# gonglixue/RAFT-tf

Hardware: AMD Instinct MI355X
Metric: frames/sec (whole node), raft-things 2x436x1024, 32 iters, inference (higher is better)
Workload: dtype bf16; 1 GPU; model=raft-things, global_batch=1, height=436, width=1024, iters=32, parallelism=dp1, device=mi355x

## Files before the change

raft_amd/models/fused.py:

```python
from __future__ import annotations

from typing import Optional

import torch

ACT_NONE, ACT_RELU, ACT_SIGMOID, ACT_TANH = 0, 1, 2, 3


def _pad8(c: int) -> int:
    return (c + 7) // 8 * 8


def pack_conv(conv: torch.nn.Conv2d, pad_cin: Optional[int] = None,
              scale: float = 1.0):
    w = conv.weight.detach().float()
    N, Cin, kh, kw = w.shape
    cp = pad_cin if pad_cin is not None else Cin
    wp = w.new_zeros(N, cp, kh, kw)
    wp[:, :Cin] = w * scale
    wp = wp.permute(2, 3, 0, 1).reshape(kh * kw, N, cp)
    wp = wp.contiguous().to(device=conv.weight.device, dtype=torch.bfloat16)
    if conv.bias is not None:
        bias = (conv.bias.detach().float() * scale).contiguous()
    else:
# ... 9 lines not shown


class _FC:

    def __init__(self, conv, pad_cin=None, scale=1.0):
        self.wp, self.bias, self.kh, self.kw = pack_conv(conv, pad_cin, scale)

    def __call__(self, hip, in1, in2=None, act=ACT_RELU, out=None, n_off=0,
                 in1_off=0, in1_len=0, stride=1, res=None):
        return hip.fconv_plain(in1, in2, self.wp, self.bias, self.kh,
                               self.kw, act, out, n_off, in1_off, in1_len,
                               -1, -1, stride, res)


class _GruDir:
    def __init__(self, convz, convr, convq):
        self.zr_w, self.zr_b, self.kh, self.kw = pack_zr(convz, convr)
        self.q_w, self.q_b, _, _ = pack_conv(convq)

    def __call__(self, hip, h, x):
        z, rh = hip.fconv_gru_zr(h, x, self.zr_w, self.zr_b, self.kh, self.kw)
        return hip.fconv_gru_q(rh, x, self.q_w, self.q_b, self.kh, self.kw,
                               z, h)


def _pack_fp8(wp_bf16, dev):
    w = wp_bf16.float()
    aw = float(w.abs().max().clamp_min(1e-12))
    w8 = (w * (448.0 / aw)).to(torch.float8_e4m3fn).view(torch.uint8)
    return w8.contiguous().to(dev), aw


class _GruDirFP8:

    def __init__(self, convz, convr, convq):
        zr_w, self.zr_b, self.kh, self.kw = pack_zr(convz, convr)
        q_w, self.q_b, _, _ = pack_conv(convq)
        dev = self.zr_b.device
        self.zr_w8, self.zr_aw = _pack_fp8(zr_w, dev)
        self.q_w8, self.q_aw = _pack_fp8(q_w, dev)

    def __call__(self, hip, h, x8, ax, h8):
        z, rh8 = hip.fconv_fp8_gru_zr(h8, x8, h, self.zr_w8, self.zr_b, ax,
                                      self.zr_aw, self.kh, self.kw)
        return hip.fconv_fp8_gru_q(rh8, x8, self.q_w8, self.q_b, ax,
                                   self.q_aw, self.kh, self.kw, z, h)


class FusedBasicUpdate:

    def __init__(self, ub, corr_cpad: int, ctx_dim: int):
        enc = ub.encoder
        self.c1 = _FC(enc.convc1, pad_cin=corr_cpad)
        self.c2 = _FC(enc.convc2)
        self.f1 = _FC(enc.convf1)
        self.f2 = _FC(enc.convf2)
        self.cv = _FC(enc.conv)
        import os as _os
        hd = ub.gru.convz1.weight.shape[0]
        cat_dim = ub.gru.convz1.weight.shape[1]
        self.fp8_gru = (_os.environ.get("RAFT_AMD_FP8_GRU", "0") == "1"
                        and hd % 128 == 0 and (cat_dim - hd) % 128 == 0)
        if self.fp8_gru:
            self.gru1 = _GruDirFP8(ub.gru.convz1, ub.gru.convr1,
                                   ub.gru.convq1)
            self.gru2 = _GruDirFP8(ub.gru.convz2, ub.gru.convr2,
                                   ub.gru.convq2)
        else:
            self.gru1 = _GruDir(ub.gru.convz1, ub.gru.convr1, ub.gru.convq1)
            self.gru2 = _GruDir(ub.gru.convz2, ub.gru.convr2, ub.gru.convq2)
        self.fh1 = _FC(ub.flow_head.conv1)
        self.m0 = _FC(ub.mask[0])
        self.heads_w = torch.cat([self.fh1.wp, self.m0.wp], dim=1) \
            .contiguous()
        self.heads_b = torch.cat([self.fh1.bias, self.m0.bias]).contiguous()
        self.fh2 = _FC(ub.flow_head.conv2)
        self.m2 = _FC(ub.mask[2], scale=0.25)
        self.ctx_dim = ctx_dim
        self.side_stream = None
        self._ev_fork = torch.cuda.Event()
        self._ev_join = torch.cuda.Event()

    def __call__(self, hip, net, x_buf, corr_pad, coords1, final=True):
        ctx = self.ctx_dim
        side = self.side_stream
        if side is not None and not torch.cuda.is_current_stream_capturing():
            cur = torch.cuda.current_stream()
            self._ev_fork.record(cur)
            side.wait_event(self._ev_fork)
            with torch.cuda.stream(side):
                flo1 = hip.fconv_smallk(x_buf, self.f1.wp, self.f1.bias,
                                        self.f1.kh, self.f1.kw, ACT_RELU,
                                        ctx + 126, 2, 1)
                flo = self.f2(hip, flo1)
                self._ev_join.record(side)
            cor = self.c2(hip, self.c1(hip, corr_pad))
            cur.wait_event(self._ev_join)
            flo.record_stream(cur)
        else:
            cor = self.c2(hip, self.c1(hip, corr_pad))
            flo1 = hip.fconv_smallk(x_buf, self.f1.wp, self.f1.bias,
                                    self.f1.kh, self.f1.kw, ACT_RELU,
                                    ctx + 126, 2, 1)
            flo = self.f2(hip, flo1)
        self.cv(hip, cor, flo, ACT_RELU, out=x_buf, n_off=ctx)
        if self.fp8_gru:
            ax = x_buf.abs().amax().to(torch.float32).clamp_(min=1.0) \
                .contiguous()
            x8 = hip.quant_fp8(x_buf, ax)
            net = self.gru1(hip, net, x8, ax, hip.quant_fp8(net, ax))
            net = self.gru2(hip, net, x8, ax, hip.quant_fp8(net, ax))
        else:
            net = self.gru1(hip, net, x_buf)
            net = self.gru2(hip, net, x_buf)
        if not final:
            h1 = self.fh1(hip, net)
            coords_new = hip.fconv_dflow_coords(h1, self.fh2.wp,
                                                self.fh2.bias, coords1, 3, 3)
            return net, None, coords_new
        hbuf = hip.fconv_plain(net, None, self.heads_w, self.heads_b, 3, 3,
                               ACT_RELU, None, 0, 0, 0, -1, -1, 1, None)
        coords_new = hip.fconv_dflow_coords(hbuf, self.fh2.wp,
                                            self.fh2.bias, coords1, 3, 3)
        mask = self.m2(hip, hbuf, act=ACT_NONE, in1_off=256, in1_len=256)
        return net, mask, coords_new


class FusedSmallUpdate:

    def __init__(self, ub, corr_cpad: int, ctx_dim: int):
        enc = ub.encoder
        self.c1 = _FC(enc.convc1, pad_cin=corr_cpad)
        self.f1 = _FC(enc.convf1)
        self.f2 = _FC(enc.convf2)
        self.cv = _FC(enc.conv)
        self.gru = _GruDir(ub.gru.convz, ub.gru.convr, ub.gru.convq)
        self.fh1 = _FC(ub.flow_head.conv1)
        self.fh2 = _FC(ub.flow_head.conv2)
        self.ctx_dim = ctx_dim
        self.side_stream = None
        self._ev_fork = torch.cuda.Event()
        self._ev_join = torch.cuda.Event()

    def __call__(self, hip, net, x_buf, corr_pad, coords1, final=True):
        ctx = self.ctx_dim
        side = self.side_stream
        if side is not None and not torch.cuda.is_current_stream_capturing():
            cur = torch.cuda.current_stream()
            self._ev_fork.record(cur)
            side.wait_event(self._ev_fork)
            with torch.cuda.stream(side):
                flo1 = hip.fconv_smallk(x_buf, self.f1.wp, self.f1.bias,
                                        self.f1.kh, self.f1.kw, ACT_RELU,
                                        ctx + 80, 2, 1)
                flo = self.f2(hip, flo1)
                self._ev_join.record(side)
            cor = self.c1(hip, corr_pad)
            cur.wait_event(self._ev_join)
            flo.record_stream(cur)
        else:
            cor = self.c1(hip, corr_pad)
            flo1 = hip.fconv_smallk(x_buf, self.f1.wp, self.f1.bias,
                                    self.f1.kh, self.f1.kw, ACT_RELU,
                                    ctx + 80, 2, 1)
            flo = self.f2(hip, flo1)
        self.cv(hip, cor, flo, ACT_RELU, out=x_buf, n_off=ctx)
        net = self.gru(hip, net, x_buf)
        h1 = self.fh1(hip, net)
        coords_new = hip.fconv_dflow_coords(h1, self.fh2.wp, self.fh2.bias,
                                            coords1, 3, 3)
        return net, None, coords_new


def pack_raw(w: torch.Tensor, bias, pad_cin: Optional[int] = None):
    N, Cin, kh, kw = w.shape
    cp = pad_cin if pad_cin is not None else Cin
    wp = w.new_zeros(N, cp, kh, kw)
    wp[:, :Cin] = w
    wp = wp.permute(2, 3, 0, 1).reshape(kh * kw, N, cp)
    wp = wp.contiguous().to(torch.bfloat16)
    if bias is None:
        bias = torch.zeros(N, device=w.device)
# ... 98 lines not shown


_warned_bidir_fp8 = False


class FusedRaft:

    def __init__(self, model):
        from raft_amd.ops import require_hip
        self.hip = require_hip()
        self.model = model
        cfg = model.cfg
        K = 2 * cfg.corr_radius + 1
        self.corr_c = cfg.corr_levels * K * K
        self.corr_cpad = _pad8(self.corr_c)
        if cfg.small:
            self.update = FusedSmallUpdate(model.update_block, self.corr_cpad,
                                           cfg.context_dim)
            self.x_dim = cfg.context_dim + 82
        else:
            self.update = FusedBasicUpdate(model.update_block, self.corr_cpad,
                                           cfg.context_dim)
            self.x_dim = cfg.context_dim + 128
        import os
        self.fuse_enc = os.environ.get("RAFT_AMD_EAGER_ENC", "0") != "1"
        if self.fuse_enc:
            fnorm = "instance"
            cnorm = "none" if cfg.small else "batch"
            self.fnet_f = FusedEncoder(model.fnet, fnorm)
            self.cnet_f = FusedEncoder(model.cnet, cnorm)
        self._version = self._weights_version()
        self._graphs = {}

    def _weights_version(self) -> int:
        return sum(p._version for p in self.model.parameters())

    def stale(self) -> bool:
        return self._version != self._weights_version()

    @torch.no_grad()
    def _loop(self, levels, net, x_buf, coords0, coords1, iters):
        cfg = self.model.cfg
        hip = self.hip
        B, H8, W8, _ = coords0.shape
        corr_buf = torch.zeros(B, H8, W8, self.corr_cpad,
                               device=net.device, dtype=torch.bfloat16)
        flow_off = self.x_dim - 2
        mask = None
        for it in range(iters):
            corr_pad = hip.corr_lookup_nhwc(list(levels), coords1,
                                            cfg.corr_radius, self.corr_cpad,
                                            True, corr_buf, x_buf, flow_off,
                                            getattr(self, "_vol_scale",
                                                    None))
            net, mask, coords1 = self.update(hip, net, x_buf, corr_pad,
                                             coords1,
                                             final=(it == iters - 1))

        flow = coords1 - coords0
        if cfg.small:
            from raft_amd.ops import torch_ref
            up = torch_ref.upflow8(flow.permute(0, 3, 1, 2))
            if cfg.scale_small_upflow:
                up = 8.0 * up
            return up, flow
        flow_nchw = flow.permute(0, 3, 1, 2).contiguous()
        mask_nchw = mask.permute(0, 3, 1, 2).contiguous()
        return hip.convex_upsample(flow_nchw, mask_nchw), flow

    def _side(self):
        side = getattr(self, "_side_stream", None)
        if side is None:
# ... 221 lines not shown
```

raft_amd/ops/csrc/bindings.cpp:

```cpp
#include <torch/extension.h>

#include <ATen/hip/HIPContext.h>
#include <c10/hip/HIPStream.h>
#include <hip/hip_runtime_api.h>

#include <cmath>
#include <vector>

extern "C" {
void launch_corr_volume_f32(const float*, const float*, float*, int, int,
                            int, int, float, hipStream_t);
void launch_corr_pool2x_f32(const float*, float*, int, int, int, int,
                            long long, hipStream_t);
void launch_corr_lookup_fwd_f32(const float* const*, const int*, const int*,
                                const float*, float*, int, int, int, int,
                                int, hipStream_t);
void launch_corr_lookup_bwd_f32(float* const*, const int*, const int*,
                                const float*, const float*, int, int, int,
                                int, int, hipStream_t);
void launch_corr_lookup_bwd_wave_f32(float* const*, const int*, const int*,
                                     const float*, const void*, int, int,
                                     int, int, int, int, int, hipStream_t);
void launch_gru_gates_fwd_f32(const float*, const float*, const float*,
                              float*, long long, hipStream_t);
// ... 43 lines not shown
int launch_frame_interp(const float*, const float*, const float*,
                        const float*, const unsigned char*,
                        const unsigned char*, unsigned long long*, float*,
                        float*, float*, unsigned char*, int, int, int, int,
                        float, hipStream_t);
void launch_corr_lookup_nhwc(const void* const*, const int*, const int*,
                             int, const float*, const float*, void*, bool,
                             void*, int, int, int, int, int, int, int, int,
                             hipStream_t);
void launch_corr_lookup_nhwc_bwd(float* const*, const int*, const int*,
                                 const float*, const float*, int, int, int,
                                 int, int, hipStream_t);
void launch_corr_pool2x_bf16(const void*, void*, int, int, int, int,
                             long long, hipStream_t);
void launch_fconv_nhwc_bf16(const void*, int, int, int, const void*, int,
                            const void*, const float*, void*, int, int, int,
                            int, int, int, int, int, int, int, const void*,
                            const void*, void*, void*, int, int, int,
                            hipStream_t);
void launch_inorm_stats(const void*, float*, float*, float*, int, int,
                        int, float, hipStream_t);
int inorm_stats_partitions(int);
void launch_inorm_apply(const void*, const float*, const float*,
                        const void*, void*, int, int, int, int,
                        hipStream_t);
void launch_fconv_smallk_nhwc_bf16(const void*, int, int, const void*,
                                   const float*, void*, int, int, int, int,
                                   int, int, int, int, int, hipStream_t);
void launch_fconv_dflow_coords(const void*, int, int, int, const void*,
                               const float*, const float*, float*, int, int,
                               int, int, int, hipStream_t);
}

// ... 626 lines not shown
        res_ptr = res->data_ptr();
        mode = 3;
    }
    at::Tensor out;
    int cstride;
    if (out_buf.has_value()) {
        out = out_buf.value();
        CHECK_CONT(out);
        cstride = out.size(3);
    } else {
        out = at::empty({B, Ho, Wo, N}, in1.options());
        cstride = N;
        n_off = 0;
    }
    launch_fconv_nhwc_bf16(in1.data_ptr(), C1, in1_stride, (int)in1_off,
                           p2, C2, wp.data_ptr(), bptr, out.data_ptr(), B,
                           Ho, Wo, N, (int)n_off, cstride, (int)kh, (int)kw,
                           (int)act, mode, res_ptr, nullptr, nullptr,
                           nullptr, (int)alltaps, (int)mtiles, (int)stride,
                           current_stream());
    return out;
}

std::vector<at::Tensor> fconv_gru_zr(at::Tensor h, at::Tensor x,
                                     at::Tensor wp, at::Tensor bias,
                                     int64_t kh, int64_t kw) {
    CHECK_DEV(h); CHECK_CONT(h); CHECK_CONT(x); CHECK_CONT(wp);
    const int B = h.size(0), H = h.size(1), W = h.size(2), hd = h.size(3);
    const int N = wp.size(1);
    TORCH_CHECK(N == 2 * hd, "zr weights must stack [Wz; Wr]");
    auto z = at::empty_like(h);
    auto rh = at::empty_like(h);
    launch_fconv_nhwc_bf16(h.data_ptr(), hd, hd, 0, x.data_ptr(),
                           x.size(3), wp.data_ptr(), bias.data_ptr<float>(),
                           nullptr, B, H, W, N, 0, 0, (int)kh, (int)kw, 0,
                           1, h.data_ptr(), nullptr, z.data_ptr(),
                           rh.data_ptr(), -1, -1, 1, current_stream());
    return {z, rh};
}

at::Tensor fconv_gru_q(at::Tensor rh, at::Tensor x, at::Tensor wp,
                       at::Tensor bias, int64_t kh, int64_t kw, at::Tensor z,
                       at::Tensor h) {
    CHECK_DEV(rh); CHECK_CONT(rh); CHECK_CONT(x); CHECK_CONT(wp);
    CHECK_CONT(z); CHECK_CONT(h);
    const int B = rh.size(0), H = rh.size(1), W = rh.size(2);
    const int hd = rh.size(3);
    TORCH_CHECK(wp.size(1) == hd);
    auto out = at::empty_like(h);
    launch_fconv_nhwc_bf16(rh.data_ptr(), hd, hd, 0, x.data_ptr(),
                           x.size(3), wp.data_ptr(),
                           bias.data_ptr<float>(), out.data_ptr(), B, H, W,
                           hd, 0, hd, (int)kh, (int)kw, 0, 2, h.data_ptr(),
                           z.data_ptr(), nullptr, nullptr, -1, -1, 1,
                           current_stream());
    return out;
}

at::Tensor fconv_smallk(at::Tensor in1, at::Tensor wp,
                        c10::optional<at::Tensor> bias, int64_t kh,
                        int64_t kw, int64_t act, int64_t in1_off,
                        int64_t in1_len, int64_t conv_stride) {
    CHECK_DEV(in1); CHECK_CONT(in1); CHECK_CONT(wp);
    const int B = in1.size(0), H = in1.size(1), W = in1.size(2);
    const int stride = in1.size(3);
    const int C = in1_len > 0 ? (int)in1_len : stride;
    const int N = wp.size(1);
    const float* bptr = bias.has_value() ? bias->data_ptr<float>() : nullptr;
    const int Ho = (int)(H / conv_stride), Wo = (int)(W / conv_stride);
    TORCH_CHECK(conv_stride == 1 ||
// ... 98 lines not shown
          py::arg("levels"), py::arg("coords"), py::arg("radius"),
          py::arg("c_stride"), py::arg("out_bf16"),
          py::arg("out_buf") = c10::nullopt,
          py::arg("flow_buf") = c10::nullopt, py::arg("flow_off") = 0,
          py::arg("vol_scale") = c10::nullopt);
    m.def("fconv_plain", &fconv_plain,
          "fused NHWC bf16 conv (+bias +activation, slice output)");
    m.def("fconv_gru_zr", &fconv_gru_zr, "GRU z/r gate conv pair");
    m.def("fconv_smallk", &fconv_smallk, "direct NHWC conv for tiny Cin");
    m.def("inorm_stats", &inorm_stats, "per-(b,c) instance-norm stats");
    m.def("inorm_apply", &inorm_apply,
          "instance-norm apply (+relu / +residual-relu)");
    m.def("fconv_dflow_coords", &fconv_dflow_coords,
          "flow-head final conv fused with the coords update");
    m.def("fconv_gru_q", &fconv_gru_q, "GRU candidate conv + state update");
}
```

raft_amd/ops/csrc/fconv.hip:

```cpp

#include "common.h"
#include "fconv_dispatch.h"
#include <hip/hip_bf16.h>
#include <cstdio>

typedef short short8 __attribute__((ext_vector_type(8)));
typedef unsigned int uint4v __attribute__((ext_vector_type(4)));

#define FC_BM 64
#define FC_BN 128
#define FC_BK 32
#define FC_ROWB (FC_BK * 2)

RAFT_DEV unsigned fswz(int row, unsigned colbyte) {
    return (unsigned)(row * FC_ROWB + colbyte) ^
           (((unsigned)row & 3u) << 4) ^ ((((unsigned)row >> 2) & 3u) << 6);
}

RAFT_DEV float factivate(float v, int act) {
    if (act == 1) return fmaxf(v, 0.0f);
    if (act == 2) return 1.0f / (1.0f + __expf(-v));
    if (act == 3) return tanhf(v);
    return v;
}

#define EP_PLAIN 0
#define EP_GRU_ZR 1
#define EP_GRU_Q 2
#define EP_RES_RELU 3

template <int KH, int KW, int MI, int NJ, bool AT, int MT, int S, int TH = 1,
          bool PIPE = false>
__global__ __launch_bounds__(256) void fconv_nhwc_bf16_k(
    const __hip_bfloat16* __restrict__ in1, int C1,
    int in1_stride, int in1_off,
    const __hip_bfloat16* __restrict__ in2, int C2,
    const __hip_bfloat16* __restrict__ wp,
    const float* __restrict__ bias,
    __hip_bfloat16* __restrict__ out,
    int H, int W, int N, int n_off, int out_cstride, int act, int mode,
    const __hip_bfloat16* __restrict__ h_state,
    const __hip_bfloat16* __restrict__ z_buf_in,
    __hip_bfloat16* __restrict__ z_buf_out,
    __hip_bfloat16* __restrict__ rh_out) {
    constexpr int TAPS = KH * KW;
    constexpr int BM = 32 * MI;
    constexpr int BN = 32 * NJ;
    constexpr int PAR = (S == 2) ? 2 : 1;
    constexpr int PBW = (S == 2) ? (KW - 2) / 2 : KW / 2;
    constexpr int PBH = (S == 2) ? (KH - 2) / 2 : KH / 2;
    constexpr int RLO = (S == 2) ? (PBW + 1) / 2 : 0;
    constexpr int BMX = BM / TH;
    constexpr int AW = (S == 2) ? (BM + RLO + (KW + 1) / 2 + 1)
                                : (BMX + KW - 1);
    constexpr int APAD = ((AW + 15) / 16) * 16;
    constexpr int NSLAB = ((AT ? KH : 1) + TH - 1) * MT * PAR;
    constexpr int NBT = AT ? TAPS : KW;
    constexpr int ABYTES = APAD * FC_ROWB;
    constexpr int BBYTES = BN * FC_ROWB;
// ... 10 lines not shown
    const int wave = tid >> 6;
    const int wm = (wave >> 1) * (16 * MI);
    const int wn = (wave & 1) * (16 * NJ);
    const long long HW = (long long)H * W;
    const int ksteps = (Cin + FC_BK - 1) / FC_BK;
    const int nsteps = AT ? ksteps : KH * ksteps;

    floatx4 acc[MT][MI][NJ];
#pragma unroll
    for (int mt = 0; mt < MT; ++mt)
#pragma unroll
        for (int i = 0; i < MI; ++i)
#pragma unroll
            for (int j = 0; j < NJ; ++j)
                acc[mt][i][j] = {0.f, 0.f, 0.f, 0.f};

    char* const sAbase = smem;
    char* const sBbase = smem + NSLAB * ABYTES;

    auto stage = [&](int s) {
        const int ty0 = AT ? 0 : s / ksteps;
        const int k0 = (AT ? s : (s - ty0 * ksteps)) * FC_BK;
        const int Hi = (S == 2) ? 2 * H : H;
        const int Wi = (S == 2) ? 2 * W : W;
        const bool a_one = (k0 + FC_BK <= C1) || (k0 >= C1);
        const bool a_rows =
            (S == 1) && (y - KH / 2 + (AT ? 0 : ty0) >= 0) &&
            (y + (AT ? KH - 1 : ty0) + TH - 1 - KH / 2 < H);
        const bool a_cols = (x0 - KW / 2 + (MT - 1) * 0 >= 0) &&
                            (x0 + MT * BMX - 1 + (KW - 1) / 2 < W);
        if (a_one && a_rows && a_cols && S == 1) {
            const bool use1 = k0 + FC_BK <= C1;
            const __hip_bfloat16* src = use1 ? in1 : in2;
            const int cs = use1 ? in1_stride : C2;
            const int co = use1 ? (in1_off + k0) : (k0 - C1);
            for (int e = tid; e < NSLAB * AW * (FC_BK / 8); e += 256) {
                const int sl = e / (AW * (FC_BK / 8));
                const int rem0 = e % (AW * (FC_BK / 8));
                const int ar = rem0 / (FC_BK / 8);
                const int c8 = (rem0 % (FC_BK / 8)) * 8;
                const int mt = (sl / PAR) % MT;
                const int rsl = sl / (PAR * MT);
                const int row = y + (ty0 + rsl) - PBH;
                const int x = x0 + mt * BMX + ar - PBW;
                const uint4v v = *(const uint4v*)(
                    src + (((long long)b * H + row) * W + x) * cs + co + c8);
                *(uint4v*)(sAbase + sl * ABYTES + fswz(ar, c8 * 2)) = v;
            }
        } else
// ... 14 lines not shown
                : (x0 + mt * BMX + ar - PBW);
            uint4v v = {0, 0, 0, 0};
            if (row_ok && x >= 0 && x < Wi) {
                const int k = k0 + c8;
                const long long p = ((long long)b * Hi + row) * Wi + x;
                if (k < C1) {
                    if (k + 8 <= C1)
                        v = *(const uint4v*)(in1 + p * in1_stride + in1_off
                                             + k);
                    else {
                        __hip_bfloat16 tmp[8];
                        for (int u = 0; u < 8; ++u) {
                            const int kk = k + u;
                            tmp[u] = (kk < C1)
                                   ? in1[p * in1_stride + in1_off + kk]
                                   : (kk - C1 < C2 ? in2[p * C2 + kk - C1]
                                                   : (__hip_bfloat16)0.f);
                        }
                        v = *(const uint4v*)tmp;
                    }
                } else if (k - C1 < C2) {
                    if (k - C1 + 8 <= C2)
                        v = *(const uint4v*)(in2 + p * C2 + (k - C1));
                    else {
                        __hip_bfloat16 tmp[8];
                        for (int u = 0; u < 8; ++u) {
                            const int kk = k - C1 + u;
                            tmp[u] = kk < C2 ? in2[p * C2 + kk]
                                             : (__hip_bfloat16)0.f;
                        }
                        v = *(const uint4v*)tmp;
                    }
                }
            }
            *(uint4v*)(sA + fswz(ar, c8 * 2)) = v;
        }
        if (n0 + BN <= N && k0 + FC_BK <= Cin) {
            for (int e = tid; e < NBT * BN * (FC_BK / 8); e += 256) {
                const int t = e / (BN * (FC_BK / 8));
                const int rem = e % (BN * (FC_BK / 8));
                const int n = rem / (FC_BK / 8);
                const int c8 = (rem % (FC_BK / 8)) * 8;
                const int tap = AT ? t : (ty0 * KW + t);
// ... 81 lines not shown

        auto loadA = [&](int s, uint4v* rg) {
            const int ty0 = AT ? 0 : s / ksteps;
            const int k0 = (AT ? s : (s - ty0 * ksteps)) * FC_BK;
            const int Hi = (S == 2) ? 2 * H : H;
            const int Wi = (S == 2) ? 2 * W : W;
            const bool a_one = (k0 + FC_BK <= C1) || (k0 >= C1);
            const bool a_rows =
                (S == 1) && (y - KH / 2 + (AT ? 0 : ty0) >= 0) &&
                (y + (AT ? KH - 1 : ty0) + TH - 1 - KH / 2 < H);
            const bool a_cols = (x0 - KW / 2 >= 0) &&
                                (x0 + MT * BMX - 1 + (KW - 1) / 2 < W);
            if (S == 1 && a_one && a_rows && a_cols) {
                const bool use1 = k0 + FC_BK <= C1;
                const __hip_bfloat16* src = use1 ? in1 : in2;
                const int cs = use1 ? in1_stride : C2;
                const int co = use1 ? (in1_off + k0) : (k0 - C1);
#pragma unroll
                for (int r = 0; r < RA; ++r) {
                    const int e = tid + r * 256;
                    if (e < TOTA) {
                        const int sl = e / (AW * (FC_BK / 8));
                        const int rem0 = e % (AW * (FC_BK / 8));
                        const int ar = rem0 / (FC_BK / 8);
                        const int c8 = (rem0 % (FC_BK / 8)) * 8;
                        const int mt = (sl / PAR) % MT;
                        const int rsl = sl / (PAR * MT);
                        const int row = y + (ty0 + rsl) - PBH;
                        const int x = x0 + mt * BMX + ar - PBW;
                        rg[r] = *(const uint4v*)(
                            src + (((long long)b * H + row) * W + x) * cs +
// ... 22 lines not shown
                        : (x0 + mt * BMX + ar - PBW);
                    if (row_ok && x >= 0 && x < Wi) {
                        const int k = k0 + c8;
                        const long long p = ((long long)b * Hi + row) * Wi + x;
                        if (k < C1) {
                            if (k + 8 <= C1)
                                v = *(const uint4v*)(
                                    in1 + p * in1_stride + in1_off + k);
                            else {
                                __hip_bfloat16 tmp[8];
                                for (int u = 0; u < 8; ++u) {
                                    const int kk = k + u;
                                    tmp[u] = (kk < C1)
                                        ? in1[p * in1_stride + in1_off + kk]
                                        : (kk - C1 < C2
                                               ? in2[p * C2 + kk - C1]
                                               : (__hip_bfloat16)0.f);
                                }
                                v = *(const uint4v*)tmp;
                            }
                        } else if (k - C1 < C2) {
                            if (k - C1 + 8 <= C2)
                                v = *(const uint4v*)(in2 + p * C2 + (k - C1));
                            else {
                                __hip_bfloat16 tmp[8];
                                for (int u = 0; u < 8; ++u) {
                                    const int kk = k - C1 + u;
                                    tmp[u] = kk < C2
                                        ? in2[p * C2 + kk]
                                        : (__hip_bfloat16)0.f;
                                }
                                v = *(const uint4v*)tmp;
                            }
                        }
                    }
                }
                rg[r] = v;
            }
        };

        auto loadB = [&](int s, uint4v* rg) {
            const int ty0 = AT ? 0 : s / ksteps;
            const int k0 = (AT ? s : (s - ty0 * ksteps)) * FC_BK;
            if (n0 + BN <= N && k0 + FC_BK <= Cin) {
// ... 92 lines not shown
                const int m = wm + i * 16 + (lane >> 4) * 4 + r;
                const int n = n0 + wn + j * 16 + (lane & 15);
                const int yy2 = y + m / BMX;
                const int x = x0 + mt * BMX + m % BMX;
                if (x >= W || n >= N || yy2 >= H) continue;
                const long long p = ((long long)b * H + yy2) * W + x;
                float v = acc[mt][i][j][r];
                if (bias) v += bias[n];
                if (mode == EP_PLAIN) {
                    out[p * out_cstride + n_off + n] =
                        (__hip_bfloat16)factivate(v, act);
                } else if (mode == EP_RES_RELU) {
                    const float res = (float)h_state[p * hd + n];
                    out[p * out_cstride + n_off + n] = (__hip_bfloat16)
                        fmaxf(res + fmaxf(v, 0.0f), 0.0f);
                } else if (mode == EP_GRU_ZR) {
                    const float s = 1.0f / (1.0f + __expf(-v));
                    if (n < hd) {
                        z_buf_out[p * hd + n] = (__hip_bfloat16)s;
                    } else {
                        const int c = n - hd;
                        rh_out[p * hd + c] = (__hip_bfloat16)(
                            s * (float)h_state[p * hd + c]);
                    }
                } else {
                    const float q = tanhf(v);
                    const float z = (float)z_buf_in[p * hd + n];
                    const float h = (float)h_state[p * hd + n];
                    out[p * out_cstride + n_off + n] =
                        (__hip_bfloat16)((1.0f - z) * h + z * q);
                }
            }
}


extern "C" __global__ __launch_bounds__(256) void fconv_stem_s2_k(
    const __hip_bfloat16* __restrict__ in,
    const __hip_bfloat16* __restrict__ wp,
    const float* __restrict__ bias,
    __hip_bfloat16* __restrict__ out,
    int H, int W, int N, int act) {
    constexpr int KT = 49, KTP = 52;
// ... 186 lines not shown
}

static const FconvKnobs& fconv_knobs() {
    static const FconvKnobs k = fconv_knobs_from_env();
    return k;
}

struct FconvArgs {
    const __hip_bfloat16 *in1, *in2, *wp;
    const float* bias;
    __hip_bfloat16* out;
    const __hip_bfloat16 *h_state, *z_buf_in;
    __hip_bfloat16 *z_buf_out, *rh_out;
    int act;
    hipStream_t s;
};

template <int KH, int KW, int MI, int NJ, bool AT, int MT, int S, int TH,
          bool PIPE>
static bool fc_try(const FconvPick& p, const FconvShape& sh,
                   const FconvArgs& a) {
    if (p.KH != KH || p.KW != KW || p.MI != MI || p.NJ != NJ ||
        (p.AT != 0) != AT || p.MT != MT || p.S != S || p.TH != TH ||
        (p.PIPE != 0) != PIPE)
        return false;
    unsigned g[3];
    fconv_generic_grid(p, sh, g);
    hipLaunchKernelGGL(
        (fconv_nhwc_bf16_k<KH, KW, MI, NJ, AT, MT, S, TH, PIPE>),
        dim3(g[0], g[1], g[2]), dim3(256), 0, a.s, a.in1, sh.C1,
        sh.in1_stride, sh.in1_off, a.in2, sh.C2, a.wp, a.bias, a.out, sh.H,
        sh.W, sh.N, sh.n_off, sh.out_cstride, a.act, sh.mode, a.h_state,
        a.z_buf_in, a.z_buf_out, a.rh_out);
    return true;
}

template <int KH, int KW, int MI, int NJ, bool AT, int MT, int S, int TH>
static bool fc_try_pp(const FconvPick& p, const FconvShape& sh,
                      const FconvArgs& a) {
    return fc_try<KH, KW, MI, NJ, AT, MT, S, TH, false>(p, sh, a) ||
           fc_try<KH, KW, MI, NJ, AT, MT, S, TH, true>(p, sh, a);
}

template <int KH, int KW>
static bool fc_try_s1(const FconvPick& p, const FconvShape& sh,
                      const FconvArgs& a) {
    if (p.S != 1 || p.KH != KH || p.KW != KW) return false;
    if (fc_try_pp<KH, KW, 2, 4, false, 1, 1, 1>(p, sh, a) ||
// ... 18 lines not shown
            fc_try_pp<KH, KW, 1, 1, true, 1, 1, 8>(p, sh, a))
            return true;
    }
    return false;
}

template <int K>
static bool fc_try_s2(const FconvPick& p, const FconvShape& sh,
                      const FconvArgs& a) {
    return fc_try<K, K, 2, 4, false, 1, 2, 1, false>(p, sh, a) ||
           fc_try<K, K, 1, 2, false, 1, 2, 1, false>(p, sh, a);
}

extern "C" void launch_fconv_nhwc_bf16(
    const void* in1, int C1, int in1_stride, int in1_off, const void* in2,
    int C2, const void* wp, const float* bias, void* out, int B, int H,
    int W, int N, int n_off, int out_cstride, int kh, int kw, int act,
    int mode, const void* h_state, const void* z_buf_in, void* z_buf_out,
    void* rh_out, int alltaps, int mtiles, int stride, hipStream_t s) {
    const FconvShape sh{B, H, W, N, C1, in1_stride, in1_off, C2,
                        in2 != nullptr, kh, kw, stride, mode, n_off,
                        out_cstride};
    const FconvPick p = fconv_pick(sh, alltaps, mtiles, fconv_knobs());
    const FconvArgs a{(const __hip_bfloat16*)in1, (const __hip_bfloat16*)in2,
                      (const __hip_bfloat16*)wp, bias, (__hip_bfloat16*)out,
                      (const __hip_bfloat16*)h_state,
                      (const __hip_bfloat16*)z_buf_in,
                      (__hip_bfloat16*)z_buf_out, (__hip_bfloat16*)rh_out,
                      act, s};
    const dim3 blk(256);
    switch (p.kind) {
    case FCONV_TINYN: {
        const long long ncells = (long long)B * H * W;
        hipLaunchKernelGGL(fconv_tinyn_k<2>, dim3((unsigned)((ncells + 3) / 4)),
                           blk, 0, s, a.in1, C1, in1_stride, in1_off, a.wp,
                           bias, a.out, nullptr, nullptr, H, W, kh, kw, act,
                           ncells);
        return;
    }
    case FCONV_TINYN2: {
        const int smem = (kh * (8 + kw - 1) * C1 + kh * kw * 2 * C1) * 2;
        hipLaunchKernelGGL(fconv_tinyn2_k<2>,
                           dim3((unsigned)(H * ((W + 7) / 8)), 1, (unsigned)B),
                           blk, smem, s, a.in1, C1, in1_stride, in1_off, a.wp,
// ... 398 lines not shown
```

Measured before the change: 113.9 frames/s.

## Hoist loop-invariant context-channel GRU convolution out of the refinement loop

Splits the GRU z/r/q convolution weights into the context-channel part, which is constant across iterations, and the per-iteration part. The context contribution plus bias is computed once before the loop into an fp32 buffer. Each iteration's GRU kernels start their accumulators from that buffer and convolve only the hidden state and motion features, which cuts the GEMM K dimension. The cost is an extra fp32 tensor read per output and more kernel arguments, and the hoist is on by default unless the fp8 GRU path is selected.

```diff
diff --git a/raft_amd/models/fused.py b/raft_amd/models/fused.py
--- a/raft_amd/models/fused.py
+++ b/raft_amd/models/fused.py
@@ -47,14 +47,36 @@
 
 
 class _GruDir:
-    def __init__(self, convz, convr, convq):
+
+    def __init__(self, convz, convr, convq, ctx: int = 0):
         self.zr_w, self.zr_b, self.kh, self.kw = pack_zr(convz, convr)
         self.q_w, self.q_b, _, _ = pack_conv(convq)
-
-    def __call__(self, hip, h, x):
-        z, rh = hip.fconv_gru_zr(h, x, self.zr_w, self.zr_b, self.kh, self.kw)
-        return hip.fconv_gru_q(rh, x, self.q_w, self.q_b, self.kh, self.kw,
-                               z, h)
+        self.ctx = ctx
+        self.hd = hd = self.q_w.shape[1]
+        if ctx:
+            full = torch.cat([self.zr_w, self.q_w], dim=1)
+            self.pre_w = full[..., hd:hd + ctx].contiguous()
+            self.pre_b = torch.cat([self.zr_b, self.q_b]).contiguous()
+            loop = torch.cat([full[..., :hd], full[..., hd + ctx:]], dim=-1)
+            self.zr_w = loop[:, :2 * hd].contiguous()
+            self.q_w = loop[:, 2 * hd:].contiguous()
+            self.zr_b = self.q_b = None
+
+    def precompute(self, hip, x):
+        return hip.fconv_plain_f32(x, self.pre_w, self.pre_b, self.kh,
+                                   self.kw, 0, self.ctx)
+
+    def __call__(self, hip, h, x, pre=None):
+        if not self.ctx:
+            z, rh = hip.fconv_gru_zr(h, x, self.zr_w, self.zr_b, self.kh,
+                                     self.kw)
+            return hip.fconv_gru_q(rh, x, self.q_w, self.q_b, self.kh,
+                                   self.kw, z, h)
+        ctx, rest = self.ctx, x.shape[-1] - self.ctx
+        z, rh = hip.fconv_gru_zr_pre(h, x, self.zr_w, self.kh, self.kw, pre,
+                                     0, ctx, rest)
+        return hip.fconv_gru_q_pre(rh, x, self.q_w, self.kh, self.kw, z, h,
+                                   pre, 2 * self.hd, ctx, rest)
 
 
 def _pack_fp8(wp_bf16, dev):
@@ -82,7 +104,7 @@
 
 class FusedBasicUpdate:
 
-    def __init__(self, ub, corr_cpad: int, ctx_dim: int):
+    def __init__(self, ub, corr_cpad: int, ctx_dim: int, hoist: bool = False):
         enc = ub.encoder
         self.c1 = _FC(enc.convc1, pad_cin=corr_cpad)
         self.c2 = _FC(enc.convc2)
@@ -100,8 +122,12 @@
             self.gru2 = _GruDirFP8(ub.gru.convz2, ub.gru.convr2,
                                    ub.gru.convq2)
         else:
-            self.gru1 = _GruDir(ub.gru.convz1, ub.gru.convr1, ub.gru.convq1)
-            self.gru2 = _GruDir(ub.gru.convz2, ub.gru.convr2, ub.gru.convq2)
+            hc = ctx_dim if hoist else 0
+            self.gru1 = _GruDir(ub.gru.convz1, ub.gru.convr1, ub.gru.convq1,
+                                hc)
+            self.gru2 = _GruDir(ub.gru.convz2, ub.gru.convr2, ub.gru.convq2,
+                                hc)
+        self.hoist = hoist and not self.fp8_gru
         self.fh1 = _FC(ub.flow_head.conv1)
         self.m0 = _FC(ub.mask[0])
         self.heads_w = torch.cat([self.fh1.wp, self.m0.wp], dim=1) \
@@ -114,7 +140,14 @@
         self._ev_fork = torch.cuda.Event()
         self._ev_join = torch.cuda.Event()
 
-    def __call__(self, hip, net, x_buf, corr_pad, coords1, final=True):
+    def precompute(self, hip, x_buf):
+        if not self.hoist:
+            return None
+        return (self.gru1.precompute(hip, x_buf),
+                self.gru2.precompute(hip, x_buf))
+
+    def __call__(self, hip, net, x_buf, corr_pad, coords1, final=True,
+                 pre=None):
         ctx = self.ctx_dim
         side = self.side_stream
         if side is not None and not torch.cuda.is_current_stream_capturing():
@@ -143,6 +176,9 @@
             x8 = hip.quant_fp8(x_buf, ax)
             net = self.gru1(hip, net, x8, ax, hip.quant_fp8(net, ax))
             net = self.gru2(hip, net, x8, ax, hip.quant_fp8(net, ax))
+        elif self.hoist:
+            net = self.gru1(hip, net, x_buf, pre[0])
+            net = self.gru2(hip, net, x_buf, pre[1])
         else:
             net = self.gru1(hip, net, x_buf)
             net = self.gru2(hip, net, x_buf)
@@ -161,13 +197,15 @@
 
 class FusedSmallUpdate:
 
-    def __init__(self, ub, corr_cpad: int, ctx_dim: int):
+    def __init__(self, ub, corr_cpad: int, ctx_dim: int, hoist: bool = False):
         enc = ub.encoder
         self.c1 = _FC(enc.convc1, pad_cin=corr_cpad)
         self.f1 = _FC(enc.convf1)
         self.f2 = _FC(enc.convf2)
         self.cv = _FC(enc.conv)
-        self.gru = _GruDir(ub.gru.convz, ub.gru.convr, ub.gru.convq)
+        self.hoist = hoist
+        self.gru = _GruDir(ub.gru.convz, ub.gru.convr, ub.gru.convq,
+                           ctx_dim if hoist else 0)
         self.fh1 = _FC(ub.flow_head.conv1)
         self.fh2 = _FC(ub.flow_head.conv2)
         self.ctx_dim = ctx_dim
@@ -175,7 +213,11 @@
         self._ev_fork = torch.cuda.Event()
         self._ev_join = torch.cuda.Event()
 
-    def __call__(self, hip, net, x_buf, corr_pad, coords1, final=True):
+    def precompute(self, hip, x_buf):
+        return self.gru.precompute(hip, x_buf) if self.hoist else None
+
+    def __call__(self, hip, net, x_buf, corr_pad, coords1, final=True,
+                 pre=None):
         ctx = self.ctx_dim
         side = self.side_stream
         if side is not None and not torch.cuda.is_current_stream_capturing():
@@ -198,7 +240,7 @@
                                     ctx + 80, 2, 1)
             flo = self.f2(hip, flo1)
         self.cv(hip, cor, flo, ACT_RELU, out=x_buf, n_off=ctx)
-        net = self.gru(hip, net, x_buf)
+        net = self.gru(hip, net, x_buf, pre)
         h1 = self.fh1(hip, net)
         coords_new = hip.fconv_dflow_coords(h1, self.fh2.wp, self.fh2.bias,
                                             coords1, 3, 3)
@@ -327,15 +369,18 @@
         K = 2 * cfg.corr_radius + 1
         self.corr_c = cfg.corr_levels * K * K
         self.corr_cpad = _pad8(self.corr_c)
+        import os
+        hoist = (os.environ.get("RAFT_AMD_GRU_HOIST", "1") != "0"
+                 and cfg.context_dim % 8 == 0)
         if cfg.small:
             self.update = FusedSmallUpdate(model.update_block, self.corr_cpad,
-                                           cfg.context_dim)
+                                           cfg.context_dim, hoist)
             self.x_dim = cfg.context_dim + 82
         else:
             self.update = FusedBasicUpdate(model.update_block, self.corr_cpad,
-                                           cfg.context_dim)
+                                           cfg.context_dim, hoist)
             self.x_dim = cfg.context_dim + 128
-        import os
+        self.gru_hoist = self.update.hoist
         self.fuse_enc = os.environ.get("RAFT_AMD_EAGER_ENC", "0") != "1"
         if self.fuse_enc:
             fnorm = "instance"
@@ -360,6 +405,7 @@
                                device=net.device, dtype=torch.bfloat16)
         flow_off = self.x_dim - 2
         mask = None
+        pre = self.update.precompute(hip, x_buf)
         for it in range(iters):
             corr_pad = hip.corr_lookup_nhwc(list(levels), coords1,
                                             cfg.corr_radius, self.corr_cpad,
@@ -368,7 +414,8 @@
                                                     None))
             net, mask, coords1 = self.update(hip, net, x_buf, corr_pad,
                                              coords1,
-                                             final=(it == iters - 1))
+                                             final=(it == iters - 1),
+                                             pre=pre)
 
         flow = coords1 - coords0
         if cfg.small:
diff --git a/raft_amd/ops/csrc/bindings.cpp b/raft_amd/ops/csrc/bindings.cpp
--- a/raft_amd/ops/csrc/bindings.cpp
+++ b/raft_amd/ops/csrc/bindings.cpp
@@ -81,9 +81,10 @@
 void launch_corr_pool2x_bf16(const void*, void*, int, int, int, int,
                              long long, hipStream_t);
 void launch_fconv_nhwc_bf16(const void*, int, int, int, const void*, int,
-                            const void*, const float*, void*, int, int, int,
-                            int, int, int, int, int, int, int, const void*,
-                            const void*, void*, void*, int, int, int,
+                            int, int, const void*, const float*, void*, int,
+                            int, int, int, int, int, int, int, int, int,
+                            const void*, const void*, void*, void*,
+                            const float*, int, int, int, int, int,
                             hipStream_t);
 void launch_inorm_stats(const void*, float*, float*, float*, int, int,
                         int, float, hipStream_t);
@@ -740,10 +741,11 @@
         n_off = 0;
     }
     launch_fconv_nhwc_bf16(in1.data_ptr(), C1, in1_stride, (int)in1_off,
-                           p2, C2, wp.data_ptr(), bptr, out.data_ptr(), B,
-                           Ho, Wo, N, (int)n_off, cstride, (int)kh, (int)kw,
-                           (int)act, mode, res_ptr, nullptr, nullptr,
-                           nullptr, (int)alltaps, (int)mtiles, (int)stride,
+                           p2, C2, C2, 0, wp.data_ptr(), bptr,
+                           out.data_ptr(), B, Ho, Wo, N, (int)n_off, cstride,
+                           (int)kh, (int)kw, (int)act, mode, res_ptr,
+                           nullptr, nullptr, nullptr, nullptr, 0, 0,
+                           (int)alltaps, (int)mtiles, (int)stride,
                            current_stream());
     return out;
 }
@@ -758,10 +760,11 @@
     auto z = at::empty_like(h);
     auto rh = at::empty_like(h);
     launch_fconv_nhwc_bf16(h.data_ptr(), hd, hd, 0, x.data_ptr(),
-                           x.size(3), wp.data_ptr(), bias.data_ptr<float>(),
-                           nullptr, B, H, W, N, 0, 0, (int)kh, (int)kw, 0,
-                           1, h.data_ptr(), nullptr, z.data_ptr(),
-                           rh.data_ptr(), -1, -1, 1, current_stream());
+                           x.size(3), x.size(3), 0, wp.data_ptr(),
+                           bias.data_ptr<float>(), nullptr, B, H, W, N, 0, 0,
+                           (int)kh, (int)kw, 0, 1, h.data_ptr(), nullptr,
+                           z.data_ptr(), rh.data_ptr(), nullptr, 0, 0, -1,
+                           -1, 1, current_stream());
     return {z, rh};
 }
 
@@ -775,11 +778,117 @@
     TORCH_CHECK(wp.size(1) == hd);
     auto out = at::empty_like(h);
     launch_fconv_nhwc_bf16(rh.data_ptr(), hd, hd, 0, x.data_ptr(),
-                           x.size(3), wp.data_ptr(),
+                           x.size(3), x.size(3), 0, wp.data_ptr(),
                            bias.data_ptr<float>(), out.data_ptr(), B, H, W,
                            hd, 0, hd, (int)kh, (int)kw, 0, 2, h.data_ptr(),
-                           z.data_ptr(), nullptr, nullptr, -1, -1, 1,
+                           z.data_ptr(), nullptr, nullptr, nullptr, 0, 0,
+                           -1, -1, 1, current_stream());
+    return out;
+}
+
+
+at::Tensor fconv_plain_f32(at::Tensor in1, at::Tensor wp,
+                           c10::optional<at::Tensor> bias, int64_t kh,
+                           int64_t kw, int64_t in1_off, int64_t in1_len) {
+    CHECK_DEV(in1); CHECK_CONT(in1); CHECK_DEV(wp); CHECK_CONT(wp);
+    TORCH_CHECK(in1.scalar_type() == at::kBFloat16 &&
+                wp.scalar_type() == at::kBFloat16, "fconv needs bf16");
+    TORCH_CHECK((kh == 1 && kw == 1) || (kh == 3 && kw == 3) ||
+                (kh == 1 && kw == 5) || (kh == 5 && kw == 1),
+                "fconv: unsupported kernel shape ", kh, "x", kw);
+    const int B = in1.size(0), H = in1.size(1), W = in1.size(2);
+    const int in1_stride = in1.size(3);
+    const int C1 = in1_len > 0 ? (int)in1_len : in1_stride;
+    TORCH_CHECK(in1_off >= 0 && in1_off % 8 == 0 &&
+                in1_off + C1 <= in1_stride, "in1 slice out of bounds or "
+                "not 16-byte aligned");
+    const int N = wp.size(1);
+    TORCH_CHECK(wp.size(0) == kh * kw && wp.size(2) == C1,
+                "packed weight shape mismatch");
+    const float* bptr = nullptr;
+    if (bias.has_value()) {
+        CHECK_DEV(bias.value()); CHECK_CONT(bias.value());
+        TORCH_CHECK(bias->scalar_type() == at::kFloat && bias->numel() == N);
+        bptr = bias->data_ptr<float>();
+    }
+    auto out = at::empty({B, H, W, N}, in1.options().dtype(at::kFloat));
+    launch_fconv_nhwc_bf16(in1.data_ptr(), C1, in1_stride, (int)in1_off,
+                           nullptr, 0, 0, 0, wp.data_ptr(), bptr,
+                           out.data_ptr(), B, H, W, N, 0, N, (int)kh, (int)kw,
+                           0, 4 , nullptr, nullptr, nullptr,
+                           nullptr, nullptr, 0, 0, -1, -1, 1,
                            current_stream());
+    return out;
+}
+
+static void check_gru_pre(const at::Tensor& h, const at::Tensor& x,
+                          const at::Tensor& wp, const at::Tensor& pre,
+                          int64_t pre_off, int64_t x_off, int64_t x_len,
+                          int64_t N) {
+    TORCH_CHECK(h.scalar_type() == at::kBFloat16 &&
+                x.scalar_type() == at::kBFloat16 &&
+                wp.scalar_type() == at::kBFloat16, "fconv needs bf16");
+    TORCH_CHECK(x.dim() == 4 && x.size(0) == h.size(0) &&
+                x.size(1) == h.size(1) && x.size(2) == h.size(2),
+                "x and h disagree in B/H/W");
+    TORCH_CHECK(x_off % 8 == 0, "x_off must be a multiple of 8 (16-byte "
+                "vector loads), got ", x_off);
+    TORCH_CHECK(x_off >= 0 && x_len > 0 && x_off + x_len <= x.size(3),
+                "x slice [", x_off, ", ", x_off + x_len, ") exceeds ",
+                x.size(3), " channels");
+    TORCH_CHECK(wp.size(2) == h.size(3) + x_len,
+                "packed weight must have hd + x_len input channels");
+    CHECK_DEV(pre);
+    TORCH_CHECK(pre.scalar_type() == at::kFloat, "pre must be fp32");
+    TORCH_CHECK(pre.is_contiguous(), "pre must be contiguous");
+    TORCH_CHECK(pre.dim() == 4 && pre.size(0) == h.size(0) &&
+                pre.size(1) == h.size(1) && pre.size(2) == h.size(2),
+                "pre and h disagree in B/H/W");
+    TORCH_CHECK(pre_off >= 0 && pre_off + N <= pre.size(3),
+                "pre_off + N = ", pre_off + N, " exceeds pre's ",
+                pre.size(3), " channels");
+}
+
+std::vector<at::Tensor> fconv_gru_zr_pre(at::Tensor h, at::Tensor x,
+                                         at::Tensor wp, int64_t kh,
+                                         int64_t kw, at::Tensor pre,
+                                         int64_t pre_off, int64_t x_off,
+                                         int64_t x_len) {
+    CHECK_DEV(h); CHECK_CONT(h); CHECK_CONT(x); CHECK_CONT(wp);
+    const int B = h.size(0), H = h.size(1), W = h.size(2), hd = h.size(3);
+    const int N = wp.size(1);
+    TORCH_CHECK(N == 2 * hd, "zr weights must stack [Wz; Wr]");
+    check_gru_pre(h, x, wp, pre, pre_off, x_off, x_len, N);
+    auto z = at::empty_like(h);
+    auto rh = at::empty_like(h);
+    launch_fconv_nhwc_bf16(h.data_ptr(), hd, hd, 0, x.data_ptr(), (int)x_len,
+                           (int)x.size(3), (int)x_off, wp.data_ptr(),
+                           nullptr, nullptr, B, H, W, N, 0, 0, (int)kh,
+                           (int)kw, 0, 1, h.data_ptr(), nullptr,
+                           z.data_ptr(), rh.data_ptr(),
+                           pre.data_ptr<float>(), (int)pre.size(3),
+                           (int)pre_off, -1, -1, 1, current_stream());
+    return {z, rh};
+}
+
+at::Tensor fconv_gru_q_pre(at::Tensor rh, at::Tensor x, at::Tensor wp,
+                           int64_t kh, int64_t kw, at::Tensor z, at::Tensor h,
+                           at::Tensor pre, int64_t pre_off, int64_t x_off,
+                           int64_t x_len) {
+    CHECK_DEV(rh); CHECK_CONT(rh); CHECK_CONT(x); CHECK_CONT(wp);
+    CHECK_CONT(z); CHECK_CONT(h);
+    const int B = rh.size(0), H = rh.size(1), W = rh.size(2);
+    const int hd = rh.size(3);
+    TORCH_CHECK(wp.size(1) == hd);
+    check_gru_pre(rh, x, wp, pre, pre_off, x_off, x_len, hd);
+    auto out = at::empty_like(h);
+    launch_fconv_nhwc_bf16(rh.data_ptr(), hd, hd, 0, x.data_ptr(),
+                           (int)x_len, (int)x.size(3), (int)x_off,
+                           wp.data_ptr(), nullptr, out.data_ptr(), B, H, W,
+                           hd, 0, hd, (int)kh, (int)kw, 0, 2, h.data_ptr(),
+                           z.data_ptr(), nullptr, nullptr,
+                           pre.data_ptr<float>(), (int)pre.size(3),
+                           (int)pre_off, -1, -1, 1, current_stream());
     return out;
 }
 
@@ -908,4 +1017,20 @@
     m.def("fconv_dflow_coords", &fconv_dflow_coords,
           "flow-head final conv fused with the coords update");
     m.def("fconv_gru_q", &fconv_gru_q, "GRU candidate conv + state update");
-}
+    m.def("fconv_plain_f32", &fconv_plain_f32,
+          "NHWC bf16 conv (+bias) with unrounded fp32 output, no activation",
+          py::arg("in1"), py::arg("wp"), py::arg("bias"), py::arg("kh"),
+          py::arg("kw"), py::arg("in1_off") = 0, py::arg("in1_len") = 0);
+    m.def("fconv_gru_zr_pre", &fconv_gru_zr_pre,
+          "GRU z/r conv pair over [h | x[..., x_off:x_off+x_len]] plus the "
+          "fp32 term pre[..., pre_off:pre_off+2*hd] (bias folded in)",
+          py::arg("h"), py::arg("x"), py::arg("wp"), py::arg("kh"),
+          py::arg("kw"), py::arg("pre"), py::arg("pre_off"),
+          py::arg("x_off"), py::arg("x_len"));
+    m.def("fconv_gru_q_pre", &fconv_gru_q_pre,
+          "GRU candidate conv + state update over [rh | x slice] plus the "
+          "fp32 term pre[..., pre_off:pre_off+hd] (bias folded in)",
+          py::arg("rh"), py::arg("x"), py::arg("wp"), py::arg("kh"),
+          py::arg("kw"), py::arg("z"), py::arg("h"), py::arg("pre"),
+          py::arg("pre_off"), py::arg("x_off"), py::arg("x_len"));
+}
diff --git a/raft_amd/ops/csrc/fconv.hip b/raft_amd/ops/csrc/fconv.hip
--- a/raft_amd/ops/csrc/fconv.hip
+++ b/raft_amd/ops/csrc/fconv.hip
@@ -28,6 +28,7 @@
 #define EP_GRU_ZR 1
 #define EP_GRU_Q 2
 #define EP_RES_RELU 3
+#define EP_PLAIN_F32 4
 
 template <int KH, int KW, int MI, int NJ, bool AT, int MT, int S, int TH = 1,
           bool PIPE = false>
@@ -35,14 +36,16 @@
     const __hip_bfloat16* __restrict__ in1, int C1,
     int in1_stride, int in1_off,
     const __hip_bfloat16* __restrict__ in2, int C2,
+    int in2_stride,
     const __hip_bfloat16* __restrict__ wp,
     const float* __restrict__ bias,
     __hip_bfloat16* __restrict__ out,
     int H, int W, int N, int n_off, int out_cstride, int act, int mode,
+    int pre_stride,
     const __hip_bfloat16* __restrict__ h_state,
-    const __hip_bfloat16* __restrict__ z_buf_in,
-    __hip_bfloat16* __restrict__ z_buf_out,
-    __hip_bfloat16* __restrict__ rh_out) {
+    __hip_bfloat16* __restrict__ z_buf,
+    __hip_bfloat16* __restrict__ rh_out,
+    const float* __restrict__ pre) {
     constexpr int TAPS = KH * KW;
     constexpr int BM = 32 * MI;
     constexpr int BN = 32 * NJ;
@@ -83,6 +86,25 @@
 #pragma unroll
             for (int j = 0; j < NJ; ++j)
                 acc[mt][i][j] = {0.f, 0.f, 0.f, 0.f};
+    if (pre) {
+#pragma unroll
+        for (int mt = 0; mt < MT; ++mt)
+#pragma unroll
+            for (int i = 0; i < MI; ++i)
+#pragma unroll
+                for (int j = 0; j < NJ; ++j)
+#pragma unroll
+                    for (int r = 0; r < 4; ++r) {
+                        const int m = wm + i * 16 + (lane >> 4) * 4 + r;
+                        const int n = n0 + wn + j * 16 + (lane & 15);
+                        const int yy2 = y + m / BMX;
+                        const int x = x0 + mt * BMX + m % BMX;
+                        if (x < W && n < N && yy2 < H)
+                            acc[mt][i][j][r] = pre[
+                                (((long long)b * H + yy2) * W + x) *
+                                pre_stride + n];
+                    }
+    }
 
     char* const sAbase = smem;
     char* const sBbase = smem + NSLAB * ABYTES;
@@ -101,7 +123,7 @@
         if (a_one && a_rows && a_cols && S == 1) {
             const bool use1 = k0 + FC_BK <= C1;
             const __hip_bfloat16* src = use1 ? in1 : in2;
-            const int cs = use1 ? in1_stride : C2;
+            const int cs = use1 ? in1_stride : in2_stride;
             const int co = use1 ? (in1_off + k0) : (k0 - C1);
             for (int e = tid; e < NSLAB * AW * (FC_BK / 8); e += 256) {
                 const int sl = e / (AW * (FC_BK / 8));
@@ -146,19 +168,21 @@
                             const int kk = k + u;
                             tmp[u] = (kk < C1)
                                    ? in1[p * in1_stride + in1_off + kk]
-                                   : (kk - C1 < C2 ? in2[p * C2 + kk - C1]
-                                                   : (__hip_bfloat16)0.f);
+                                   : (kk - C1 < C2
+                                          ? in2[p * in2_stride + kk - C1]
+                                          : (__hip_bfloat16)0.f);
                         }
                         v = *(const uint4v*)tmp;
                     }
                 } else if (k - C1 < C2) {
                     if (k - C1 + 8 <= C2)
-                        v = *(const uint4v*)(in2 + p * C2 + (k - C1));
+                        v = *(const uint4v*)(in2 + p * in2_stride
+                                             + (k - C1));
                     else {
                         __hip_bfloat16 tmp[8];
                         for (int u = 0; u < 8; ++u) {
                             const int kk = k - C1 + u;
-                            tmp[u] = kk < C2 ? in2[p * C2 + kk]
+                            tmp[u] = kk < C2 ? in2[p * in2_stride + kk]
                                              : (__hip_bfloat16)0.f;
                         }
                         v = *(const uint4v*)tmp;
@@ -270,7 +294,7 @@
             if (S == 1 && a_one && a_rows && a_cols) {
                 const bool use1 = k0 + FC_BK <= C1;
                 const __hip_bfloat16* src = use1 ? in1 : in2;
-                const int cs = use1 ? in1_stride : C2;
+                const int cs = use1 ? in1_stride : in2_stride;
                 const int co = use1 ? (in1_off + k0) : (k0 - C1);
 #pragma unroll
                 for (int r = 0; r < RA; ++r) {
@@ -323,20 +347,21 @@
                                     tmp[u] = (kk < C1)
                                         ? in1[p * in1_stride + in1_off + kk]
                                         : (kk - C1 < C2
-                                               ? in2[p * C2 + kk - C1]
+                                               ? in2[p * in2_stride + kk - C1]
                                                : (__hip_bfloat16)0.f);
                                 }
                                 v = *(const uint4v*)tmp;
                             }
                         } else if (k - C1 < C2) {
                             if (k - C1 + 8 <= C2)
-                                v = *(const uint4v*)(in2 + p * C2 + (k - C1));
+                                v = *(const uint4v*)(
+                                    in2 + p * in2_stride + (k - C1));
                             else {
                                 __hip_bfloat16 tmp[8];
                                 for (int u = 0; u < 8; ++u) {
                                     const int kk = k - C1 + u;
                                     tmp[u] = kk < C2
-                                        ? in2[p * C2 + kk]
+                                        ? in2[p * in2_stride + kk]
                                         : (__hip_bfloat16)0.f;
                                 }
                                 v = *(const uint4v*)tmp;
@@ -459,10 +484,12 @@
                     const float res = (float)h_state[p * hd + n];
                     out[p * out_cstride + n_off + n] = (__hip_bfloat16)
                         fmaxf(res + fmaxf(v, 0.0f), 0.0f);
+                } else if (mode == EP_PLAIN_F32) {
+                    ((float*)out)[p * out_cstride + n_off + n] = v;
                 } else if (mode == EP_GRU_ZR) {
                     const float s = 1.0f / (1.0f + __expf(-v));
                     if (n < hd) {
-                        z_buf_out[p * hd + n] = (__hip_bfloat16)s;
+                        z_buf[p * hd + n] = (__hip_bfloat16)s;
                     } else {
                         const int c = n - hd;
                         rh_out[p * hd + c] = (__hip_bfloat16)(
@@ -470,7 +497,7 @@
                     }
                 } else {
                     const float q = tanhf(v);
-                    const float z = (float)z_buf_in[p * hd + n];
+                    const float z = (float)z_buf[p * hd + n];
                     const float h = (float)h_state[p * hd + n];
                     out[p * out_cstride + n_off + n] =
                         (__hip_bfloat16)((1.0f - z) * h + z * q);
@@ -687,6 +714,9 @@
     __hip_bfloat16 *z_buf_out, *rh_out;
     int act;
     hipStream_t s;
+    int in2_stride;
+    const float* pre;
+    int pre_stride;
 };
 
 template <int KH, int KW, int MI, int NJ, bool AT, int MT, int S, int TH,
@@ -702,9 +732,12 @@
     hipLaunchKernelGGL(
         (fconv_nhwc_bf16_k<KH, KW, MI, NJ, AT, MT, S, TH, PIPE>),
         dim3(g[0], g[1], g[2]), dim3(256), 0, a.s, a.in1, sh.C1,
-        sh.in1_stride, sh.in1_off, a.in2, sh.C2, a.wp, a.bias, a.out, sh.H,
-        sh.W, sh.N, sh.n_off, sh.out_cstride, a.act, sh.mode, a.h_state,
-        a.z_buf_in, a.z_buf_out, a.rh_out);
+        sh.in1_stride, sh.in1_off, a.in2, sh.C2, a.in2_stride, a.wp, a.bias,
+        a.out, sh.H, sh.W, sh.N, sh.n_off, sh.out_cstride, a.act, sh.mode,
+        a.pre_stride, a.h_state,
+        sh.mode == EP_GRU_ZR ? a.z_buf_out
+                             : const_cast<__hip_bfloat16*>(a.z_buf_in),
+        a.rh_out, a.pre);
     return true;
 }
 
@@ -753,20 +786,24 @@
 
 extern "C" void launch_fconv_nhwc_bf16(
     const void* in1, int C1, int in1_stride, int in1_off, const void* in2,
-    int C2, const void* wp, const float* bias, void* out, int B, int H,
-    int W, int N, int n_off, int out_cstride, int kh, int kw, int act,
-    int mode, const void* h_state, const void* z_buf_in, void* z_buf_out,
-    void* rh_out, int alltaps, int mtiles, int stride, hipStream_t s) {
+    int C2, int in2_stride, int in2_off, const void* wp, const float* bias,
+    void* out, int B, int H, int W, int N, int n_off, int out_cstride,
+    int kh, int kw, int act, int mode, const void* h_state,
+    const void* z_buf_in, void* z_buf_out, void* rh_out, const float* pre,
+    int pre_stride, int pre_off, int alltaps, int mtiles, int stride,
+    hipStream_t s) {
     const FconvShape sh{B, H, W, N, C1, in1_stride, in1_off, C2,
                         in2 != nullptr, kh, kw, stride, mode, n_off,
                         out_cstride};
     const FconvPick p = fconv_pick(sh, alltaps, mtiles, fconv_knobs());
-    const FconvArgs a{(const __hip_bfloat16*)in1, (const __hip_bfloat16*)in2,
+    const FconvArgs a{(const __hip_bfloat16*)in1,
+                      in2 ? (const __hip_bfloat16*)in2 + in2_off : nullptr,
                       (const __hip_bfloat16*)wp, bias, (__hip_bfloat16*)out,
                       (const __hip_bfloat16*)h_state,
                       (const __hip_bfloat16*)z_buf_in,
                       (__hip_bfloat16*)z_buf_out, (__hip_bfloat16*)rh_out,
-                      act, s};
+                      act, s, in2_stride, pre ? pre + pre_off : nullptr,
+                      pre_stride};
     const dim3 blk(256);
     switch (p.kind) {
     case FCONV_TINYN: {
```

Result: faster. 120.5 frames/s, median of 6 (+5.8%).
